# BolinLai/CSTS

Measured on AMD Instinct MI355X. Metric: clips/sec training (fwd+bwd) CSTS-Ego4D 16x256^2 bf16, higher is better.
Workload: dtype bf16; 1 GPU; CSTS_Ego4D_Gaze_Forecast.yaml train step (fwd + KLDiv + 0.05*EgoNCE + bwd + clip + AdamW), 16x256^2 video + 24 kHz STFT audio, b=4/GPU; mode=train, global_batch=4, frames=16, crop=256, parallelism=dp1, step=hip_graph, hip_graph=True, rccl_ranks=1

## Files before the change

### csts_amd/csrc/common.h

```cpp
#pragma once
#include <hip/hip_runtime.h>
#include <stdint.h>
#include <stddef.h>
#include <string>

#include "../../include/csts_hip.h"

#ifdef CSTS_HALF_F16
typedef _Float16 bf16;
typedef _Float16 bf16x8 __attribute__((ext_vector_type(8)));
typedef _Float16 bf16x4 __attribute__((ext_vector_type(4)));
typedef _Float16 bf16x2 __attribute__((ext_vector_type(2)));
#define CSTS_MFMA16 __builtin_amdgcn_mfma_f32_32x32x16_f16
#else
typedef __bf16 bf16;
typedef __bf16 bf16x8 __attribute__((ext_vector_type(8)));
typedef __bf16 bf16x4 __attribute__((ext_vector_type(4)));
typedef __bf16 bf16x2 __attribute__((ext_vector_type(2)));
#define CSTS_MFMA16 __builtin_amdgcn_mfma_f32_32x32x16_bf16
#endif
typedef short s16x4 __attribute__((ext_vector_type(4)));
typedef float f32x16 __attribute__((ext_vector_type(16)));
typedef float f32x4 __attribute__((ext_vector_type(4)));
typedef float f32x2 __attribute__((ext_vector_type(2)));

#define WAVE 64

__device__ __forceinline__ f32x4 ld_stream(const f32x4* p) {
#ifdef CSTS_NO_STREAM_POLICY
  return *p;
#else
  return __builtin_nontemporal_load(p);
#endif
}
__device__ __forceinline__ bf16x4 ld_stream(const bf16x4* p) {
#ifdef CSTS_NO_STREAM_POLICY
  return *p;
#else
  return __builtin_nontemporal_load(p);
#endif
}
__device__ __forceinline__ bf16x8 ld_stream(const bf16x8* p) {
#ifdef CSTS_NO_STREAM_POLICY
  return *p;
#else
  return __builtin_nontemporal_load(p);
#endif
}
typedef unsigned u32x4_t __attribute__((ext_vector_type(4)));
typedef unsigned u32x2_t __attribute__((ext_vector_type(2)));
struct StreamOut {
  __amdgpu_buffer_rsrc_t rsrc;
  __device__ __forceinline__ StreamOut(void* base, int64_t bytes) : rsrc(__builtin_amdgcn_make_buffer_rsrc(base, 0, (int)bytes, 0x00020000)) {}
  __device__ __forceinline__ void st16(int off, f32x4 v) const {
#ifdef CSTS_NO_STREAM_POLICY
    __builtin_amdgcn_raw_buffer_store_b128(__builtin_bit_cast(u32x4_t, v), rsrc, off, 0, 0);
#else
    __builtin_amdgcn_raw_buffer_store_b128(__builtin_bit_cast(u32x4_t, v), rsrc, off, 0, 17);
#endif
  }
  __device__ __forceinline__ void st8(int off, bf16x4 v) const {
#ifdef CSTS_NO_STREAM_POLICY
    __builtin_amdgcn_raw_buffer_store_b64(__builtin_bit_cast(u32x2_t, v), rsrc, off, 0, 0);
#else
    __builtin_amdgcn_raw_buffer_store_b64(__builtin_bit_cast(u32x2_t, v), rsrc, off, 0, 17);
#endif
  }
};

__device__ __forceinline__ float h16_lo(unsigned v) {
#ifdef CSTS_HALF_F16
  return (float)__builtin_bit_cast(_Float16, (unsigned short)(v & 0xffffu));
#else
  return __uint_as_float(v << 16);
#endif
}
__device__ __forceinline__ float h16_hi(unsigned v) {
#ifdef CSTS_HALF_F16
  return (float)__builtin_bit_cast(_Float16, (unsigned short)(v >> 16));
#else
  return __uint_as_float(v & 0xffff0000u);
#endif
}

void csts_set_error(const std::string& s);
#define CSTS_FAIL(msg)                                                         \
  do {                                                                         \
    csts_set_error(std::string(__func__) + ": " + (msg));                      \
    return -1;                                                                 \
  } while (0)
#define CSTS_REQUIRE(cond, msg)                                                \
  do {                                                                         \
    if (!(cond)) CSTS_FAIL(std::string(msg) + " [" #cond "]");                 \
  } while (0)
#define CSTS_LAUNCH_CHECK()                                                    \
  do {                                                                         \
    hipError_t e__ = hipGetLastError();                                        \
    if (e__ != hipSuccess) CSTS_FAIL(std::string("launch: ") + hipGetErrorString(e__)); \
  } while (0)

#include <map>
#include <mutex>
#include <utility>
static inline bool csts_dyn_lds_optin(const void* fn, int bytes) {
  static std::mutex mu;
  static std::map<std::pair<const void*, int>, int> done;
  int dev = 0;
  if (hipGetDevice(&dev) != hipSuccess) return false;
  std::lock_guard<std::mutex> lock(mu);
  auto it = done.find({fn, dev});
  if (it != done.end() && it->second >= bytes) return true;
  if (hipFuncSetAttribute(fn, hipFuncAttributeMaxDynamicSharedMemorySize, bytes) != hipSuccess) return false;
  done[{fn, dev}] = bytes;
  return true;
}

static inline bool aligned16(const void* p) { return (reinterpret_cast<uintptr_t>(p) & 15) == 0; }
static inline int64_t cdiv(int64_t a, int64_t b) { return (a + b - 1) / b; }

__device__ __forceinline__ float ld_as_f32(const void* p, int dt, int64_t i) {
  return dt == CSTS_F32 ? reinterpret_cast<const float*>(p)[i] : (float)reinterpret_cast<const bf16*>(p)[i];
}
__device__ __forceinline__ void st_from_f32(void* p, int dt, int64_t i, float v) {
  if (dt == CSTS_F32) reinterpret_cast<float*>(p)[i] = v;
  else reinterpret_cast<bf16*>(p)[i] = (bf16)v;
}

__device__ __forceinline__ void ld8_as_f32(const void* p, int dt, int64_t i, float (&o)[8]) {
  if (dt == CSTS_F32) {
    const float4* q = reinterpret_cast<const float4*>(reinterpret_cast<const float*>(p) + i);
    float4 a = q[0], b = q[1];
    o[0] = a.x; o[1] = a.y; o[2] = a.z; o[3] = a.w; o[4] = b.x; o[5] = b.y; o[6] = b.z; o[7] = b.w;
  } else {
    bf16x8 v = *reinterpret_cast<const bf16x8*>(reinterpret_cast<const bf16*>(p) + i);
#pragma unroll
    for (int j = 0; j < 8; ++j) o[j] = (float)v[j];
  }
}
__device__ __forceinline__ void st8_from_f32(void* p, int dt, int64_t i, const float (&o)[8]) {
  if (dt == CSTS_F32) {
    float4* q = reinterpret_cast<float4*>(reinterpret_cast<float*>(p) + i);
    q[0] = make_float4(o[0], o[1], o[2], o[3]);
    q[1] = make_float4(o[4], o[5], o[6], o[7]);
  } else {
    bf16x8 v;
#pragma unroll
    for (int j = 0; j < 8; ++j) v[j] = (bf16)o[j];
    *reinterpret_cast<bf16x8*>(reinterpret_cast<bf16*>(p) + i) = v;
  }
}

__device__ __forceinline__ float wave_sum(float v) {
#pragma unroll
  for (int o = 32; o > 0; o >>= 1) v += __shfl_xor(v, o, 64);
  return v;
}
__device__ __forceinline__ float wave_max(float v) {
#pragma unroll
  for (int o = 32; o > 0; o >>= 1) v = fmaxf(v, __shfl_xor(v, o, 64));
  return v;
}

__device__ __forceinline__ float gelu_f(float x) { return 0.5f * x * (1.0f + erff(x * 0.70710678118654752f)); }
__device__ __forceinline__ float dgelu_f(float x) {
  const float cdf = 0.5f * (1.0f + erff(x * 0.70710678118654752f));
  const float pdf = 0.39894228040143268f * __expf(-0.5f * x * x);
  return cdf + x * pdf;
}

__device__ __forceinline__ float erf_poly_times_exp(float ax, float e) {
  const float t = __builtin_amdgcn_rcpf(1.f + 0.3275911f * ax);
  const float poly = t * (0.254829592f + t * (-0.284496736f + t * (1.421413741f + t * (-1.453152027f + t * 1.061405429f))));
  return 1.f - poly * e;
}
__device__ __forceinline__ float gelu_fast(float x) {
  const float t = x * 0.70710678118654752f, ax = fabsf(t);
  const float e = __expf(-ax * ax);
  const float er = copysignf(erf_poly_times_exp(ax, e), x);
  return 0.5f * x * (1.0f + er);
}
__device__ __forceinline__ float dgelu_fast(float x) {
  const float t = x * 0.70710678118654752f, ax = fabsf(t);
  const float e = __expf(-ax * ax);
  const float er = copysignf(erf_poly_times_exp(ax, e), x);
  return 0.5f * (1.0f + er) + x * 0.39894228040143268f * e;
}

int csts_reduce_rows_launch(const float* ws, float* out, int64_t nrows, int64_t ncols, float scale, hipStream_t s);
```

### csts_amd/csrc/optim.hip

```cpp
#include "common.h"
#include <algorithm>
#include <type_traits>

namespace {

constexpr int OPT_THREADS = 256;
constexpr int OPT_VEC = 4;

struct OptTables {
  const int32_t* chunk_tensor;
  const int64_t* chunk_off;
  const csts_opt_tensor* tensors;
  const void* const* grads;
};

template <bool G16> __device__ __forceinline__ float ldg(const void* g, int64_t i) {
  if constexpr (G16) return (float)reinterpret_cast<const bf16*>(g)[i];
  else return reinterpret_cast<const float*>(g)[i];
}
template <bool G16> __device__ __forceinline__ float4 ldg4(const void* g, int64_t i4) {
  if constexpr (G16) {
    const bf16x4 v = ld_stream(reinterpret_cast<const bf16x4*>(g) + i4);
    return make_float4((float)v[0], (float)v[1], (float)v[2], (float)v[3]);
  } else {
    const f32x4 v = ld_stream(reinterpret_cast<const f32x4*>(g) + i4);
    return make_float4(v[0], v[1], v[2], v[3]);
  }
}
__device__ __forceinline__ float4 ld4s(const float* p, int64_t i4) {
  const f32x4 v = ld_stream(reinterpret_cast<const f32x4*>(p) + i4);
  return make_float4(v[0], v[1], v[2], v[3]);
}

template <bool G16>
__global__ __launch_bounds__(OPT_THREADS) void opt_sqnorm_kernel(OptTables t, int chunk_elems, float* __restrict__ partial,
                                                                 const float* __restrict__ scaler) {
  __shared__ float red[OPT_THREADS / WAVE];
  const int c = blockIdx.x;
  const int ti = t.chunk_tensor[c];
  const int64_t off = t.chunk_off[c];
  const char* g = reinterpret_cast<const char*>(t.grads[ti]);
  const float inv = scaler != nullptr ? 1.f / scaler[0] : 1.f;
  float s = 0.f;
  if (g != nullptr) {
    const int64_t n = min((int64_t)chunk_elems, t.tensors[ti].n - off);
    g += off * (G16 ? 2 : 4);
    const bool vec = (reinterpret_cast<uintptr_t>(g) & (G16 ? 7 : 15)) == 0;
    if (vec) {
      const int64_t n4 = n / OPT_VEC;
      for (int64_t i = threadIdx.x; i < n4; i += OPT_THREADS) {
        float4 v = ldg4<G16>(g, i);
        v.x *= inv; v.y *= inv; v.z *= inv; v.w *= inv;
        s += v.x * v.x + v.y * v.y + v.z * v.z + v.w * v.w;
      }
      for (int64_t i = n4 * OPT_VEC + threadIdx.x; i < n; i += OPT_THREADS) { const float x = ldg<G16>(g, i) * inv; s += x * x; }
    } else {
      for (int64_t i = threadIdx.x; i < n; i += OPT_THREADS) { const float x = ldg<G16>(g, i) * inv; s += x * x; }
    }
  }
  s = wave_sum(s);
  if ((threadIdx.x & 63) == 0) red[threadIdx.x >> 6] = s;
  __syncthreads();
  if (threadIdx.x == 0) {
    float tot = 0.f;
#pragma unroll
    for (int w = 0; w < OPT_THREADS / WAVE; ++w) tot += red[w];
    partial[c] = tot;
  }
}

__global__ __launch_bounds__(1024) void opt_norm_finish_kernel(const float* __restrict__ partial, int nchunks, float max_norm,
                                                               float* __restrict__ state, float* __restrict__ scaler, float growth,
                                                               float backoff, int growth_interval, const float* __restrict__ extra_sq,
                                                               int n_extra) {
  __shared__ float red[1024 / WAVE];
  float s = 0.f;
  for (int i = threadIdx.x; i < nchunks; i += 1024) s += partial[i];
  if (extra_sq != nullptr && (int)threadIdx.x < n_extra) {
    const float inv = scaler != nullptr ? 1.f / scaler[0] : 1.f;
    s += extra_sq[threadIdx.x] * inv * inv;
  }
  s = wave_sum(s);
  if ((threadIdx.x & 63) == 0) red[threadIdx.x >> 6] = s;
  __syncthreads();
  if (threadIdx.x == 0) {
    float tot = 0.f;
#pragma unroll
    for (int w = 0; w < 1024 / WAVE; ++w) tot += red[w];
    const float norm = sqrtf(tot);
    state[1] = norm;
    if (scaler != nullptr) {
      const float scale = scaler[0];
      const bool bad = !(norm == norm) || norm > 3.0e38f;
      if (bad) {
        state[2] = 0.f;
        state[3] = 1.f;
        scaler[0] = scale * backoff;
        scaler[1] = 0.f;
        return;
      }
      float tracker = scaler[1] + 1.f;
      if (tracker >= (float)growth_interval) { scaler[0] = scale * growth; tracker = 0.f; }
      scaler[1] = tracker;
      state[0] += 1.f;
      state[3] = 0.f;
      state[2] = (max_norm > 0.f ? fminf(1.f, max_norm / (norm + 1e-6f)) : 1.f) / scale;
      return;
    }
    state[0] += 1.f;
    state[3] = 0.f;
    state[2] = max_norm > 0.f ? fminf(1.f, max_norm / (norm + 1e-6f)) : 1.f;
  }
}

__device__ __forceinline__ void adamw_one(float& p, float g, float& m, float& v, float clip, float lr, float wd, float b1,
                                          float b2, float eps, float step_size, float rsqrt_bc2) {
  g *= clip;
  p -= lr * wd * p;
  m += (1.f - b1) * (g - m);
  v = b2 * v + (1.f - b2) * g * g;
  const float denom = sqrtf(v) * rsqrt_bc2 + eps;
  p -= step_size * (m / denom);
}

struct RuleK {
  float momentum, dampening;
  float clip_value;
  int nesterov;
  float* buf_step;
};

template <int R, bool VC>
__device__ __forceinline__ void rule_one(float& p, float g, float& m, float& v, float clip, float lr, float wd, float b1, float b2, float eps,
                                         float step_size, float rsqrt_bc2, const RuleK& r, bool first) {
  g *= clip;
  if constexpr (VC) g = g < -r.clip_value ? -r.clip_value : (g > r.clip_value ? r.clip_value : g);
  if constexpr (R == CSTS_OPT_ADAMW) {
    adamw_one(p, g, m, v, 1.f, lr, wd, b1, b2, eps, step_size, rsqrt_bc2);
  } else if constexpr (R == CSTS_OPT_ADAM) {
    g += wd * p;
    m += (1.f - b1) * (g - m);
    v = b2 * v + (1.f - b2) * g * g;
    const float denom = sqrtf(v) * rsqrt_bc2 + eps;
    p -= step_size * (m / denom);
  } else {
    float d = g + wd * p;
    if (r.momentum != 0.f) {
      m = first ? d : r.momentum * m + (1.f - r.dampening) * d;
      d = r.nesterov ? d + r.momentum * m : m;
    }
    p -= lr * d;
  }
}

template <int R> __device__ __forceinline__ bool rule_first(const RuleK& r, int ti, float step) {
  if constexpr (R != CSTS_OPT_SGD) return false;
  if (r.momentum == 0.f) return false;
  const float f = r.buf_step[ti];
  return f == 0.f || f == step;
}
template <int R> __device__ __forceinline__ void rule_mark(const RuleK& r, int ti, float step, bool first, bool leader) {
  if constexpr (R == CSTS_OPT_SGD) {
    if (first && leader) r.buf_step[ti] = step;
  }
}

template <bool G16, int R, bool VC>
__global__ __launch_bounds__(OPT_THREADS) void opt_adamw_kernel(OptTables t, int chunk_elems, const float* __restrict__ lr_ptr,
                                                                const float* __restrict__ state, float b1, float b2, float eps, RuleK rk) {
  const int c = blockIdx.x;
  const int ti = t.chunk_tensor[c];
  const char* g = reinterpret_cast<const char*>(t.grads[ti]);
  if (g == nullptr || state[3] != 0.f) return;
  const csts_opt_tensor tt = t.tensors[ti];
  const int64_t off = t.chunk_off[c];
  const int64_t n = min((int64_t)chunk_elems, tt.n - off);
  const float lr = *lr_ptr, step = state[0], clip = state[2];
  const float bc1 = 1.f - powf(b1, step), bc2 = 1.f - powf(b2, step);
  const float step_size = lr / bc1, rsqrt_bc2 = 1.f / sqrtf(bc2);
  constexpr bool USE_V = R != CSTS_OPT_SGD;
  const bool use_m = R != CSTS_OPT_SGD || rk.momentum != 0.f;
  if ((use_m && tt.m == nullptr) || (USE_V && tt.v == nullptr)) return;
  const bool first = rule_first<R>(rk, ti, step);
  float* p = reinterpret_cast<float*>(tt.p) + off;
  float* m = use_m ? reinterpret_cast<float*>(tt.m) + off : nullptr;
  float* v = USE_V ? reinterpret_cast<float*>(tt.v) + off : nullptr;
  bf16* w16 = tt.w16 ? reinterpret_cast<bf16*>(tt.w16) + off : nullptr;
  g += off * (G16 ? 2 : 4);
  const bool vec = ((reinterpret_cast<uintptr_t>(p) | reinterpret_cast<uintptr_t>(m) | reinterpret_cast<uintptr_t>(v)) & 15) == 0 &&
                   (reinterpret_cast<uintptr_t>(g) & (G16 ? 7 : 15)) == 0 && (w16 == nullptr || (reinterpret_cast<uintptr_t>(w16) & 7) == 0);
  int64_t done = 0;
  if (vec) {
    const int64_t n4 = n / OPT_VEC;
    const StreamOut sp(p, n * 4), sm(m ? (void*)m : (void*)p, n * 4), sv(v ? (void*)v : (void*)p, n * 4),
        sw(w16 ? (void*)w16 : (void*)p, n * 2);
    auto f4 = [](const float4& x) { f32x4 o; o[0] = x.x; o[1] = x.y; o[2] = x.z; o[3] = x.w; return o; };
    for (int64_t i = threadIdx.x; i < n4; i += OPT_THREADS) {
      float4 pp = ld4s(p, i);
      const float4 gg = ldg4<G16>(g, i);
      float4 mm = make_float4(0.f, 0.f, 0.f, 0.f), vv = mm;
      if (use_m && !first) mm = ld4s(m, i);
      if (USE_V) vv = ld4s(v, i);
      rule_one<R, VC>(pp.x, gg.x, mm.x, vv.x, clip, lr, tt.weight_decay, b1, b2, eps, step_size, rsqrt_bc2, rk, first);
      rule_one<R, VC>(pp.y, gg.y, mm.y, vv.y, clip, lr, tt.weight_decay, b1, b2, eps, step_size, rsqrt_bc2, rk, first);
      rule_one<R, VC>(pp.z, gg.z, mm.z, vv.z, clip, lr, tt.weight_decay, b1, b2, eps, step_size, rsqrt_bc2, rk, first);
      rule_one<R, VC>(pp.w, gg.w, mm.w, vv.w, clip, lr, tt.weight_decay, b1, b2, eps, step_size, rsqrt_bc2, rk, first);
      sp.st16((int)i * 16, f4(pp));
      if (use_m) sm.st16((int)i * 16, f4(mm));
      if (USE_V) sv.st16((int)i * 16, f4(vv));
      if (w16) {
        bf16x4 w;
        w[0] = (bf16)pp.x; w[1] = (bf16)pp.y; w[2] = (bf16)pp.z; w[3] = (bf16)pp.w;
        sw.st8((int)i * 8, w);
      }
    }
    done = n4 * OPT_VEC;
  }
  for (int64_t i = done + threadIdx.x; i < n; i += OPT_THREADS) {
    float pp = p[i], mm = use_m && !first ? m[i] : 0.f, vv = USE_V ? v[i] : 0.f;
    rule_one<R, VC>(pp, ldg<G16>(g, i), mm, vv, clip, lr, tt.weight_decay, b1, b2, eps, step_size, rsqrt_bc2, rk, first);
    p[i] = pp;
    if (use_m) m[i] = mm;
    if (USE_V) v[i] = vv;
    if (w16) w16[i] = (bf16)pp;
  }
  rule_mark<R>(rk, ti, step, first, off == 0 && threadIdx.x == 0);
}


constexpr int FK = 256;
constexpr int FT = 64;
constexpr int FMAX = 8;

struct FactoredList { csts_opt_factored it[FMAX]; int64_t ws_off[FMAX]; };

__device__ __forceinline__ float ld_a(const void* a, int a_dt, int64_t i) {
  return a_dt == CSTS_F32 ? reinterpret_cast<const float*>(a)[i] : (float)reinterpret_cast<const bf16*>(a)[i];
}

__global__ __launch_bounds__(256) void factored_gram_kernel(FactoredList l, float* __restrict__ ws) {
  extern __shared__ __attribute__((aligned(16))) float fsm[];
  float (*As)[FK + 1] = reinterpret_cast<float (*)[FK + 1]>(fsm);
  const csts_opt_factored& it = l.it[blockIdx.z];
  const int nslab = it.K / FK;
  if ((int)blockIdx.x >= nslab) return;
  const int k0 = blockIdx.x * FK, T = it.T;
  for (int i = threadIdx.x; i < T * (FK / 8); i += 256) {
    const int t = i / (FK / 8), k = (i - t * (FK / 8)) * 8;
    float v[8];
    ld8_as_f32(it.a, it.a_dt, (int64_t)t * it.K + k0 + k, v);
#pragma unroll
    for (int j = 0; j < 8; ++j) As[t][k + j] = v[j];
  }
  __syncthreads();
  float* out = ws + l.ws_off[blockIdx.z] + (int64_t)blockIdx.x * T * T;
  for (int pr = threadIdx.x; pr < T * T; pr += 256) {
    const int t = pr / T, u = pr - t * T;
    float s = 0.f;
#pragma unroll 8
    for (int k = 0; k < FK; ++k) s += As[t][k] * As[u][k];
    out[pr] = s;
  }
}
constexpr int FPARTS = 32;
__global__ __launch_bounds__(1024) void factored_sq_part_kernel(FactoredList l, const float* __restrict__ ws, float* __restrict__ parts) {
  const csts_opt_factored& it = l.it[blockIdx.y];
  const int T = it.T, nslab = it.K / FK, b = blockIdx.x;
  const float* w = ws + l.ws_off[blockIdx.y];
  float* out = parts + ((int64_t)blockIdx.y * FPARTS + b) * 2 * FT * FT;
  const int nb = (it.N + FPARTS - 1) / FPARTS, n_beg = b * nb, n_end = min(it.N, n_beg + nb);
  for (int pr = threadIdx.x; pr < T * T; pr += 1024) {
    const int t = pr / T, u = pr - t * T;
    float g2 = 0.f;
    for (int s = b; s < nslab; s += FPARTS) g2 += w[(int64_t)s * T * T + pr];
    float g1 = 0.f;
    if (it.a_dt == CSTS_F32) {
      for (int n = n_beg; n < n_end; ++n) g1 += it.dy[(int64_t)t * it.N + n] * it.dy[(int64_t)u * it.N + n];
    } else {
      for (int n = n_beg; n < n_end; ++n) g1 += (float)(bf16)it.dy[(int64_t)t * it.N + n] * (float)(bf16)it.dy[(int64_t)u * it.N + n];
    }
    out[pr] = g2;
    out[FT * FT + pr] = g1;
  }
}
__global__ __launch_bounds__(1024) void factored_sq_finish_kernel(FactoredList l, const float* __restrict__ parts, float* __restrict__ out_sq) {
  __shared__ float red[1024 / WAVE];
  const csts_opt_factored& it = l.it[blockIdx.x];
  const int T = it.T;
  const float* w = parts + (int64_t)blockIdx.x * FPARTS * 2 * FT * FT;
  float acc = 0.f;
  for (int pr = threadIdx.x; pr < T * T; pr += 1024) {
    float g2 = 0.f, g1 = 0.f;
    for (int b = 0; b < FPARTS; ++b) { g2 += w[(int64_t)b * 2 * FT * FT + pr]; g1 += w[(int64_t)b * 2 * FT * FT + FT * FT + pr]; }
    acc += g1 * g2;
  }
  acc = wave_sum(acc);
  if ((threadIdx.x & 63) == 0) red[threadIdx.x >> 6] = acc;
  __syncthreads();
  if (threadIdx.x == 0) {
    float tot = 0.f;
#pragma unroll
    for (int i = 0; i < 1024 / WAVE; ++i) tot += red[i];
    out_sq[blockIdx.x] = (tot == tot) ? fmaxf(tot, 0.f) : __builtin_inff();
  }
}
constexpr int FR = 32;
template <int R, bool VC>
__global__ __launch_bounds__(256) void opt_adamw_factored_kernel(FactoredList l, const float* __restrict__ lr_ptr,
                                                                 const float* __restrict__ state, float b1, float b2, float eps, RuleK rk) {
  extern __shared__ __attribute__((aligned(16))) float fsm[];
  if (state[3] != 0.f) return;
  const csts_opt_factored& it = l.it[blockIdx.z];
  float (*As)[FK] = reinterpret_cast<float (*)[FK]>(fsm);
  float (*Ds)[FR] = reinterpret_cast<float (*)[FR]>(fsm + it.T * FK);
  const int k0 = blockIdx.x * FK, n0 = blockIdx.y * FR, T = it.T;
  if (k0 >= it.K || n0 >= it.N) return;
  for (int i = threadIdx.x; i < T * (FK / 8); i += 256) {
    const int t = i / (FK / 8), k = (i - t * (FK / 8)) * 8;
    float v[8];
    ld8_as_f32(it.a, it.a_dt, (int64_t)t * it.K + k0 + k, v);
    *reinterpret_cast<float4*>(&As[t][k]) = make_float4(v[0], v[1], v[2], v[3]);
    *reinterpret_cast<float4*>(&As[t][k + 4]) = make_float4(v[4], v[5], v[6], v[7]);
  }
  for (int i = threadIdx.x; i < T * FR; i += 256) {
    const int t = i / FR, n = i - t * FR;
    Ds[t][n] = (n0 + n < it.N) ? it.dy[(int64_t)t * it.N + n0 + n] : 0.f;
  }
  __syncthreads();
  const float lr = *lr_ptr, step = state[0], clip = state[2];
  const float bc1 = 1.f - powf(b1, step), bc2 = 1.f - powf(b2, step);
  const float step_size = lr / bc1, rsqrt_bc2 = 1.f / sqrtf(bc2);
  const bool use_m = R != CSTS_OPT_SGD || rk.momentum != 0.f;
  constexpr bool USE_V = R != CSTS_OPT_SGD;
  const bool first = rule_first<R>(rk, it.tensor, step);
  const int kq = (threadIdx.x & 63) * 4;
  const int nr = threadIdx.x >> 6;
  constexpr int RPT = FR / 4;
  float g[RPT][4];
#pragma unroll
  for (int rr = 0; rr < RPT; ++rr) { g[rr][0] = 0.f; g[rr][1] = 0.f; g[rr][2] = 0.f; g[rr][3] = 0.f; }
  for (int t = 0; t < T; ++t) {
    const float4 av = *reinterpret_cast<const float4*>(&As[t][kq]);
#pragma unroll
    for (int rr = 0; rr < RPT; ++rr) {
      const float d = Ds[t][nr + 4 * rr];
      g[rr][0] += d * av.x; g[rr][1] += d * av.y; g[rr][2] += d * av.z; g[rr][3] += d * av.w;
    }
  }
#pragma unroll
  for (int rr = 0; rr < RPT; ++rr) {
    const int n = n0 + nr + 4 * rr;
    if (n >= it.N) continue;
    const int64_t at = (int64_t)n * it.K + k0 + kq;
    float4 pp = *reinterpret_cast<float4*>(it.p + at), mm = make_float4(0.f, 0.f, 0.f, 0.f), vv = mm;
    if (use_m && !first) mm = *reinterpret_cast<float4*>(it.m + at);
    if (USE_V) vv = *reinterpret_cast<float4*>(it.v + at);
    rule_one<R, VC>(pp.x, g[rr][0], mm.x, vv.x, clip, lr, it.weight_decay, b1, b2, eps, step_size, rsqrt_bc2, rk, first);
    rule_one<R, VC>(pp.y, g[rr][1], mm.y, vv.y, clip, lr, it.weight_decay, b1, b2, eps, step_size, rsqrt_bc2, rk, first);
    rule_one<R, VC>(pp.z, g[rr][2], mm.z, vv.z, clip, lr, it.weight_decay, b1, b2, eps, step_size, rsqrt_bc2, rk, first);
    rule_one<R, VC>(pp.w, g[rr][3], mm.w, vv.w, clip, lr, it.weight_decay, b1, b2, eps, step_size, rsqrt_bc2, rk, first);
    *reinterpret_cast<float4*>(it.p + at) = pp;
    if (use_m) *reinterpret_cast<float4*>(it.m + at) = mm;
    if (USE_V) *reinterpret_cast<float4*>(it.v + at) = vv;
    if (it.w16 != nullptr) {
      bf16x4 w;
      w[0] = (bf16)pp.x; w[1] = (bf16)pp.y; w[2] = (bf16)pp.z; w[3] = (bf16)pp.w;
      *reinterpret_cast<bf16x4*>(reinterpret_cast<bf16*>(it.w16) + at) = w;
    }
  }
  rule_mark<R>(rk, it.tensor, step, first, blockIdx.x == 0 && blockIdx.y == 0 && threadIdx.x == 0);
}

template <int R, bool VC>
__global__ __launch_bounds__(256) void opt_adamw_factored_mfma_kernel(FactoredList l, const float* __restrict__ lr_ptr,
                                                                      const float* __restrict__ state, float b1, float b2, float eps, RuleK rk) {
  if (state[3] != 0.f) return;
  const csts_opt_factored& it = l.it[blockIdx.z];
  const int lane = threadIdx.x & 63, wave = threadIdx.x >> 6;
  const int n0 = blockIdx.y * 32, k0 = blockIdx.x * FK + wave * 64;
  if (k0 >= it.K || n0 >= it.N) return;
  const int T = it.T, N = it.N, K = it.K;
  const bf16* __restrict__ a16 = reinterpret_cast<const bf16*>(it.a);
  f32x16 acc[2];
#pragma unroll
  for (int j = 0; j < 2; ++j)
#pragma unroll
    for (int r = 0; r < 16; ++r) acc[j][r] = 0.f;
  const int nl = n0 + (lane & 31), kl = k0 + (lane & 31);
  for (int t0 = 0; t0 < T; t0 += 16) {
    bf16x8 dv, a0, a1;
#pragma unroll
    for (int e = 0; e < 8; ++e) {
      const int t = t0 + 8 * (lane >> 5) + e;
      const bool ok = t < T;
      dv[e] = (bf16)((ok && nl < N) ? it.dy[(int64_t)t * N + nl] : 0.f);
      a0[e] = ok ? a16[(int64_t)t * K + kl] : (bf16)0.f;
      a1[e] = ok ? a16[(int64_t)t * K + kl + 32] : (bf16)0.f;
    }
    acc[0] = CSTS_MFMA16(dv, a0, acc[0], 0, 0, 0);
    acc[1] = CSTS_MFMA16(dv, a1, acc[1], 0, 0, 0);
  }
  const float lr = *lr_ptr, step = state[0], clip = state[2];
  const float bc1 = 1.f - powf(b1, step), bc2 = 1.f - powf(b2, step);
  const float step_size = lr / bc1, rsqrt_bc2 = 1.f / sqrtf(bc2);
#ifdef CSTS_NO_STREAM_POLICY
  constexpr int LD_AUX = 0, ST_AUX = 0;
#else
  constexpr int LD_AUX = 2, ST_AUX = 17;
#endif
  const bool use_m = R != CSTS_OPT_SGD || rk.momentum != 0.f;
  constexpr bool USE_V = R != CSTS_OPT_SGD;
  const bool first = rule_first<R>(rk, it.tensor, step);
  const int bytes = (int)((int64_t)N * K * 4);
  const auto rp = __builtin_amdgcn_make_buffer_rsrc(it.p, 0, bytes, 0x00020000),
             rm = __builtin_amdgcn_make_buffer_rsrc(use_m ? (void*)it.m : (void*)it.p, 0, bytes, 0x00020000),
             rv = __builtin_amdgcn_make_buffer_rsrc(USE_V ? (void*)it.v : (void*)it.p, 0, bytes, 0x00020000),
             rw = __builtin_amdgcn_make_buffer_rsrc(it.w16 != nullptr ? it.w16 : (void*)it.p, 0, bytes / 2, 0x00020000);
#pragma unroll
  for (int j = 0; j < 2; ++j) {
    float pp[16], mm[16], vv[16];
#pragma unroll
    for (int r = 0; r < 16; ++r) {
      const int n = n0 + (r & 3) + 8 * (r >> 2) + 4 * (lane >> 5);
      const int off = (n < N) ? (n * K + kl + 32 * j) * 4 : 0;
      pp[r] = __builtin_bit_cast(float, __builtin_amdgcn_raw_buffer_load_b32(rp, off, 0, LD_AUX));
      mm[r] = use_m && !first ? __builtin_bit_cast(float, __builtin_amdgcn_raw_buffer_load_b32(rm, off, 0, LD_AUX)) : 0.f;
      vv[r] = USE_V ? __builtin_bit_cast(float, __builtin_amdgcn_raw_buffer_load_b32(rv, off, 0, LD_AUX)) : 0.f;
    }
#pragma unroll
    for (int r = 0; r < 16; ++r) {
      const int n = n0 + (r & 3) + 8 * (r >> 2) + 4 * (lane >> 5);
      if (n >= N) continue;
      const int off = (n * K + kl + 32 * j) * 4;
      rule_one<R, VC>(pp[r], acc[j][r], mm[r], vv[r], clip, lr, it.weight_decay, b1, b2, eps, step_size, rsqrt_bc2, rk, first);
      __builtin_amdgcn_raw_buffer_store_b32(__builtin_bit_cast(unsigned, pp[r]), rp, off, 0, ST_AUX);
      if (use_m) __builtin_amdgcn_raw_buffer_store_b32(__builtin_bit_cast(unsigned, mm[r]), rm, off, 0, ST_AUX);
      if (USE_V) __builtin_amdgcn_raw_buffer_store_b32(__builtin_bit_cast(unsigned, vv[r]), rv, off, 0, ST_AUX);
      if (it.w16 != nullptr) __builtin_amdgcn_raw_buffer_store_b16(__builtin_bit_cast(unsigned short, (bf16)pp[r]), rw, off / 2, 0, ST_AUX);
    }
  }
  rule_mark<R>(rk, it.tensor, step, first, blockIdx.x == 0 && blockIdx.y == 0 && threadIdx.x == 0);
}

}

constexpr int FT_MFMA = 256;
static int factored_fill(const csts_opt_factored* items, int nitems, FactoredList& l, int* max_k, int* max_n, int max_t = FT,
                         bool need_m = true, bool need_v = true) {
  CSTS_REQUIRE(items != nullptr && nitems > 0 && nitems <= FMAX, "1 .. 8 items per call");
  *max_k = 0; *max_n = 0;
  int64_t off = 0;
  for (int i = 0; i < nitems; ++i) {
    const csts_opt_factored& it = items[i];
    CSTS_REQUIRE(it.p && (it.m || !need_m) && (it.v || !need_v) && it.dy && it.a, "null pointer");
    CSTS_REQUIRE(it.T > 0 && it.T <= max_t && it.K > 0 && it.K % FK == 0 && it.N > 0 && it.N % 16 == 0,
                 "T <= 64 (256 for the update with 16-bit operands), K % 256 == 0, N % 16 == 0");
    CSTS_REQUIRE(it.a_dt == CSTS_F32 || it.a_dt == CSTS_HALF, "bad a dtype");
    CSTS_REQUIRE(aligned16(it.p) && (!need_m || aligned16(it.m)) && (!need_v || aligned16(it.v)) && (it.w16 == nullptr || ((uintptr_t)it.w16 & 7) == 0), "alignment");
    l.it[i] = it;
    l.ws_off[i] = off;
    off += (int64_t)(it.K / FK) * it.T * it.T;
    *max_k = std::max(*max_k, it.K); *max_n = std::max(*max_n, it.N);
  }
  return 0;
}

extern "C" size_t csts_factored_sqnorm_workspace(const csts_opt_factored* items, int nitems) {
  if (items == nullptr || nitems <= 0 || nitems > FMAX) return 0;
  size_t b = 0;
  for (int i = 0; i < nitems; ++i) b += (size_t)(items[i].K / FK) * items[i].T * items[i].T * sizeof(float);
  return b + (size_t)nitems * FPARTS * 2 * FT * FT * sizeof(float);
}
extern "C" int csts_factored_sqnorm(const csts_opt_factored* items, int nitems, float* out_sq, void* workspace, size_t ws_bytes,
                                    hipStream_t stream) {
  FactoredList l;
  int mk, mn;
  if (int rc = factored_fill(items, nitems, l, &mk, &mn, FT, false, false)) return rc;
  CSTS_REQUIRE(out_sq != nullptr && workspace != nullptr && aligned16(workspace) && ws_bytes >= csts_factored_sqnorm_workspace(items, nitems), "workspace too small");
  float* slabs = reinterpret_cast<float*>(workspace);
  int mt = 0;
  for (int i = 0; i < nitems; ++i) mt = std::max(mt, items[i].T);
  const size_t sm = (size_t)mt * (FK + 1) * sizeof(float);
  CSTS_REQUIRE(sm <= 64 * 1024 || csts_dyn_lds_optin(reinterpret_cast<const void*>(&factored_gram_kernel), (int)sm), "LDS opt-in failed");
  hipLaunchKernelGGL(factored_gram_kernel, dim3((unsigned)(mk / FK), 1, (unsigned)nitems), dim3(256), sm, stream, l, slabs);
  CSTS_LAUNCH_CHECK();
  size_t slab_floats = 0;
  for (int i = 0; i < nitems; ++i) slab_floats += (size_t)(items[i].K / FK) * items[i].T * items[i].T;
  float* parts = slabs + slab_floats;
  hipLaunchKernelGGL(factored_sq_part_kernel, dim3(FPARTS, (unsigned)nitems), dim3(1024), 0, stream, l, (const float*)slabs, parts);
  CSTS_LAUNCH_CHECK();
  hipLaunchKernelGGL(factored_sq_finish_kernel, dim3((unsigned)nitems), dim3(1024), 0, stream, l, (const float*)parts, out_sq);
  CSTS_LAUNCH_CHECK();
  return 0;
}
static int rule_check(const csts_opt_rule* rule, RuleK* rk) {
  CSTS_REQUIRE(rule != nullptr, "null rule");
  CSTS_REQUIRE(rule->kind == CSTS_OPT_ADAMW || rule->kind == CSTS_OPT_ADAM || rule->kind == CSTS_OPT_SGD, "bad rule kind");
  CSTS_REQUIRE(rule->kind == CSTS_OPT_SGD || (rule->momentum == 0.f && rule->dampening == 0.f && rule->nesterov == 0),
               "momentum / dampening / nesterov belong to the SGD rule");
  CSTS_REQUIRE(rule->momentum >= 0.f && rule->dampening >= 0.f && rule->dampening <= 1.f, "bad momentum / dampening");
  CSTS_REQUIRE(!rule->nesterov || (rule->momentum > 0.f && rule->dampening == 0.f), "nesterov needs momentum and zero dampening");
  CSTS_REQUIRE(rule->clip_value == rule->clip_value, "bad clip_value");
  const bool sgd_m = rule->kind == CSTS_OPT_SGD && rule->momentum != 0.f;
  CSTS_REQUIRE(!sgd_m || rule->buf_step != nullptr, "SGD with momentum needs buf_step");
  *rk = RuleK{rule->momentum, rule->dampening, rule->clip_value > 0.f ? rule->clip_value : 0.f, rule->nesterov ? 1 : 0,
              sgd_m ? rule->buf_step : nullptr};
  return 0;
}
static bool rule_uses_m(const csts_opt_rule* rule) { return rule->kind != CSTS_OPT_SGD || rule->momentum != 0.f; }
static bool rule_uses_v(const csts_opt_rule* rule) { return rule->kind != CSTS_OPT_SGD; }

template <typename K3> static void launch_rule(int kind, bool vc, K3 k) {
  using VT = std::true_type;
  using VF = std::false_type;
  if (kind == CSTS_OPT_ADAMW) vc ? k(std::integral_constant<int, CSTS_OPT_ADAMW>{}, VT{}) : k(std::integral_constant<int, CSTS_OPT_ADAMW>{}, VF{});
  else if (kind == CSTS_OPT_ADAM) vc ? k(std::integral_constant<int, CSTS_OPT_ADAM>{}, VT{}) : k(std::integral_constant<int, CSTS_OPT_ADAM>{}, VF{});
  else vc ? k(std::integral_constant<int, CSTS_OPT_SGD>{}, VT{}) : k(std::integral_constant<int, CSTS_OPT_SGD>{}, VF{});
}

extern "C" int csts_opt_factored_step(const csts_opt_factored* items, int nitems, const csts_opt_rule* rule, const float* state,
                                      const float* lr, float beta1, float beta2, float eps, hipStream_t stream) {
  RuleK rk;
  if (int rc = rule_check(rule, &rk)) return rc;
  FactoredList l;
  int mk, mn;
  bool half_ops = items != nullptr && nitems > 0 && nitems <= FMAX;
  for (int i = 0; half_ops && i < nitems; ++i) half_ops = items[i].a_dt == CSTS_HALF && (int64_t)items[i].N * items[i].K * 4 < ((int64_t)1 << 31) && items[i].K % 64 == 0;
  if (int rc = factored_fill(items, nitems, l, &mk, &mn, half_ops ? FT_MFMA : FT, rule_uses_m(rule), rule_uses_v(rule))) return rc;
  CSTS_REQUIRE(state != nullptr && lr != nullptr, "null state");
  for (int i = 0; i < nitems; ++i) CSTS_REQUIRE(items[i].tensor >= 0, "bad item tensor index");
  int mt = 0;
  for (int i = 0; i < nitems; ++i) mt = std::max(mt, items[i].T);
  bool all16 = true;
  for (int i = 0; i < nitems; ++i) all16 = all16 && items[i].a_dt == CSTS_HALF && (int64_t)items[i].N * items[i].K * 4 < ((int64_t)1 << 31) && items[i].K % 64 == 0;
  if (all16) {
    launch_rule(rule->kind, rk.clip_value > 0.f, [&](auto R, auto V) {
      hipLaunchKernelGGL((opt_adamw_factored_mfma_kernel<decltype(R)::value, decltype(V)::value>), dim3((unsigned)(mk / FK), (unsigned)cdiv(mn, 32), (unsigned)nitems),
                         dim3(256), 0, stream, l, lr, state, beta1, beta2, eps, rk);
    });
    CSTS_LAUNCH_CHECK();
    return 0;
  }
  const size_t sm = (size_t)mt * (FK + FR) * sizeof(float);
  int rc = 0;
  launch_rule(rule->kind, rk.clip_value > 0.f, [&](auto R, auto V) {
    const void* fn = reinterpret_cast<const void*>(&opt_adamw_factored_kernel<decltype(R)::value, decltype(V)::value>);
    if (sm > 64 * 1024 && !csts_dyn_lds_optin(fn, (int)sm)) { rc = -1; return; }
    hipLaunchKernelGGL((opt_adamw_factored_kernel<decltype(R)::value, decltype(V)::value>), dim3((unsigned)(mk / FK), (unsigned)cdiv(mn, FR), (unsigned)nitems), dim3(256), sm,
                       stream, l, lr, state, beta1, beta2, eps, rk);
  });
  CSTS_REQUIRE(rc == 0, "LDS opt-in failed");
  CSTS_LAUNCH_CHECK();
  return 0;
}
extern "C" int csts_adamw_factored(const csts_opt_factored* items, int nitems, const float* state, const float* lr, float beta1,
                                   float beta2, float eps, hipStream_t stream) {
  const csts_opt_rule rule{CSTS_OPT_ADAMW, 0.f, 0.f, 0, 0.f, 0, nullptr};
  return csts_opt_factored_step(items, nitems, &rule, state, lr, beta1, beta2, eps, stream);
}

extern "C" int csts_opt_step(const csts_opt_args* a, const csts_opt_rule* rule, hipStream_t stream) {
  RuleK rk;
  if (int rc = rule_check(rule, &rk)) return rc;
  CSTS_REQUIRE(a != nullptr, "null args");
  CSTS_REQUIRE(a->nchunks > 0 && a->ntensors > 0 && a->chunk_elems > 0 && a->chunk_elems % 4 == 0 && a->chunk_elems <= (1 << 28), "bad chunking");
  CSTS_REQUIRE(a->chunk_tensor && a->chunk_off && a->tensors && a->grads, "null table");
  CSTS_REQUIRE(a->partial && a->state && a->lr, "null state");
  CSTS_REQUIRE(a->beta1 >= 0.f && a->beta1 < 1.f && a->beta2 >= 0.f && a->beta2 < 1.f && a->eps > 0.f, "bad hyper-parameters");
  CSTS_REQUIRE(a->grad_dt == CSTS_F32 || a->grad_dt == CSTS_HALF, "bad gradient dtype");
  CSTS_REQUIRE(a->n_extra_sq >= 0 && a->n_extra_sq <= 1024 && (a->n_extra_sq == 0 || a->extra_sq != nullptr), "bad extra_sq");
  CSTS_REQUIRE(a->scaler == nullptr || (a->growth > 1.f && a->backoff > 0.f && a->backoff < 1.f && a->growth_interval > 0), "bad loss-scaler parameters");
  CSTS_REQUIRE(!(rule->clip_value > 0.f && a->max_grad_norm > 0.f), "clip_value and max_grad_norm are exclusive (the reference's if / elif)");
  OptTables t{a->chunk_tensor, a->chunk_off, a->tensors, a->grads};
  const bool g16 = a->grad_dt != CSTS_F32;
  const dim3 grid((unsigned)a->nchunks), block(OPT_THREADS);
  if (g16) hipLaunchKernelGGL(opt_sqnorm_kernel<true>, grid, block, 0, stream, t, a->chunk_elems, a->partial, (const float*)a->scaler);
  else hipLaunchKernelGGL(opt_sqnorm_kernel<false>, grid, block, 0, stream, t, a->chunk_elems, a->partial, (const float*)a->scaler);
  CSTS_LAUNCH_CHECK();
  hipLaunchKernelGGL(opt_norm_finish_kernel, dim3(1), dim3(1024), 0, stream, a->partial, a->nchunks, a->max_grad_norm, a->state,
                     a->scaler, a->growth, a->backoff, a->growth_interval, a->extra_sq, a->n_extra_sq);
  CSTS_LAUNCH_CHECK();
  launch_rule(rule->kind, rk.clip_value > 0.f, [&](auto R, auto V) {
    constexpr int RR = decltype(R)::value;
    constexpr bool VV = decltype(V)::value;
    if (g16) hipLaunchKernelGGL((opt_adamw_kernel<true, RR, VV>), grid, block, 0, stream, t, a->chunk_elems, a->lr, a->state, a->beta1, a->beta2, a->eps, rk);
    else hipLaunchKernelGGL((opt_adamw_kernel<false, RR, VV>), grid, block, 0, stream, t, a->chunk_elems, a->lr, a->state, a->beta1, a->beta2, a->eps, rk);
  });
  CSTS_LAUNCH_CHECK();
  return 0;
}
extern "C" int csts_adamw_step(const csts_opt_args* a, hipStream_t stream) {
  const csts_opt_rule rule{CSTS_OPT_ADAMW, 0.f, 0.f, 0, 0.f, 0, nullptr};
  return csts_opt_step(a, &rule, stream);
}
```

Baseline: 206.7 clips/s.

## Add streaming factored AdamW kernel with LDS transpose and vectorized state I/O

Adds a new fused factored-gradient AdamW kernel, enabled by default, that transposes the MFMA accumulator through LDS. This lets each lane load and store param, m, v in 16-byte vector rows instead of scalar 4-byte accesses. It issues half the state loads before the MFMA loop, software-pipelines the operand loads across iterations, and pins occupancy at three waves per EU. It also relaxes the N alignment requirement to 8 and adds compile-time diagnostic switches to the old kernel. The cost is 32KB of LDS per block and higher register pressure. The optimizer is a small share of the whole training step.

After: 208.2 clips/s, median of 6. Within noise of the previous version (+0.7%).

```diff
diff --git a/csts_amd/csrc/common.h b/csts_amd/csrc/common.h
--- a/csts_amd/csrc/common.h
+++ b/csts_amd/csrc/common.h
@@ -57,6 +57,13 @@
     __builtin_amdgcn_raw_buffer_store_b128(__builtin_bit_cast(u32x4_t, v), rsrc, off, 0, 0);
 #else
     __builtin_amdgcn_raw_buffer_store_b128(__builtin_bit_cast(u32x4_t, v), rsrc, off, 0, 17);
+#endif
+  }
+  __device__ __forceinline__ f32x4 ld16(int off) const {
+#ifdef CSTS_NO_STREAM_POLICY
+    return __builtin_bit_cast(f32x4, __builtin_amdgcn_raw_buffer_load_b128(rsrc, off, 0, 0));
+#else
+    return __builtin_bit_cast(f32x4, __builtin_amdgcn_raw_buffer_load_b128(rsrc, off, 0, 2));
 #endif
   }
   __device__ __forceinline__ void st8(int off, bf16x4 v) const {
diff --git a/csts_amd/csrc/optim.hip b/csts_amd/csrc/optim.hip
--- a/csts_amd/csrc/optim.hip
+++ b/csts_amd/csrc/optim.hip
@@ -371,6 +371,9 @@
   rule_mark<R>(rk, it.tensor, step, first, blockIdx.x == 0 && blockIdx.y == 0 && threadIdx.x == 0);
 }
 
+#ifndef CSTS_FACT_DIAG
+#define CSTS_FACT_DIAG 0
+#endif
 template <int R, bool VC>
 __global__ __launch_bounds__(256) void opt_adamw_factored_mfma_kernel(FactoredList l, const float* __restrict__ lr_ptr,
                                                                       const float* __restrict__ state, float b1, float b2, float eps, RuleK rk) {
@@ -387,19 +390,6 @@
 #pragma unroll
     for (int r = 0; r < 16; ++r) acc[j][r] = 0.f;
   const int nl = n0 + (lane & 31), kl = k0 + (lane & 31);
-  for (int t0 = 0; t0 < T; t0 += 16) {
-    bf16x8 dv, a0, a1;
-#pragma unroll
-    for (int e = 0; e < 8; ++e) {
-      const int t = t0 + 8 * (lane >> 5) + e;
-      const bool ok = t < T;
-      dv[e] = (bf16)((ok && nl < N) ? it.dy[(int64_t)t * N + nl] : 0.f);
-      a0[e] = ok ? a16[(int64_t)t * K + kl] : (bf16)0.f;
-      a1[e] = ok ? a16[(int64_t)t * K + kl + 32] : (bf16)0.f;
-    }
-    acc[0] = CSTS_MFMA16(dv, a0, acc[0], 0, 0, 0);
-    acc[1] = CSTS_MFMA16(dv, a1, acc[1], 0, 0, 0);
-  }
   const float lr = *lr_ptr, step = state[0], clip = state[2];
   const float bc1 = 1.f - powf(b1, step), bc2 = 1.f - powf(b2, step);
   const float step_size = lr / bc1, rsqrt_bc2 = 1.f / sqrtf(bc2);
@@ -416,16 +406,48 @@
              rm = __builtin_amdgcn_make_buffer_rsrc(use_m ? (void*)it.m : (void*)it.p, 0, bytes, 0x00020000),
              rv = __builtin_amdgcn_make_buffer_rsrc(USE_V ? (void*)it.v : (void*)it.p, 0, bytes, 0x00020000),
              rw = __builtin_amdgcn_make_buffer_rsrc(it.w16 != nullptr ? it.w16 : (void*)it.p, 0, bytes / 2, 0x00020000);
+#if CSTS_FACT_DIAG & 4
+  float hp[2][16], hm[2][16], hv[2][16];
+#pragma unroll
+  for (int j = 0; j < 2; ++j)
+#pragma unroll
+    for (int r = 0; r < 16; ++r) {
+      const int n = n0 + (r & 3) + 8 * (r >> 2) + 4 * (lane >> 5);
+      const int off = (n < N) ? (n * K + kl + 32 * j) * 4 : 0;
+      hp[j][r] = __builtin_bit_cast(float, __builtin_amdgcn_raw_buffer_load_b32(rp, off, 0, LD_AUX));
+      hm[j][r] = use_m && !first ? __builtin_bit_cast(float, __builtin_amdgcn_raw_buffer_load_b32(rm, off, 0, LD_AUX)) : 0.f;
+      hv[j][r] = USE_V ? __builtin_bit_cast(float, __builtin_amdgcn_raw_buffer_load_b32(rv, off, 0, LD_AUX)) : 0.f;
+    }
+#endif
+#if !(CSTS_FACT_DIAG & 1)
+  for (int t0 = 0; t0 < T; t0 += 16) {
+    bf16x8 dv, a0, a1;
+#pragma unroll
+    for (int e = 0; e < 8; ++e) {
+      const int t = t0 + 8 * (lane >> 5) + e;
+      const bool ok = t < T;
+      dv[e] = (bf16)((ok && nl < N) ? it.dy[(int64_t)t * N + nl] : 0.f);
+      a0[e] = ok ? a16[(int64_t)t * K + kl] : (bf16)0.f;
+      a1[e] = ok ? a16[(int64_t)t * K + kl + 32] : (bf16)0.f;
+    }
+    acc[0] = CSTS_MFMA16(dv, a0, acc[0], 0, 0, 0);
+    acc[1] = CSTS_MFMA16(dv, a1, acc[1], 0, 0, 0);
+  }
+#endif
 #pragma unroll
   for (int j = 0; j < 2; ++j) {
     float pp[16], mm[16], vv[16];
 #pragma unroll
     for (int r = 0; r < 16; ++r) {
+#if CSTS_FACT_DIAG & 4
+      pp[r] = hp[j][r]; mm[r] = hm[j][r]; vv[r] = hv[j][r];
+#else
       const int n = n0 + (r & 3) + 8 * (r >> 2) + 4 * (lane >> 5);
       const int off = (n < N) ? (n * K + kl + 32 * j) * 4 : 0;
       pp[r] = __builtin_bit_cast(float, __builtin_amdgcn_raw_buffer_load_b32(rp, off, 0, LD_AUX));
       mm[r] = use_m && !first ? __builtin_bit_cast(float, __builtin_amdgcn_raw_buffer_load_b32(rm, off, 0, LD_AUX)) : 0.f;
       vv[r] = USE_V ? __builtin_bit_cast(float, __builtin_amdgcn_raw_buffer_load_b32(rv, off, 0, LD_AUX)) : 0.f;
+#endif
     }
 #pragma unroll
     for (int r = 0; r < 16; ++r) {
@@ -436,7 +458,102 @@
       __builtin_amdgcn_raw_buffer_store_b32(__builtin_bit_cast(unsigned, pp[r]), rp, off, 0, ST_AUX);
       if (use_m) __builtin_amdgcn_raw_buffer_store_b32(__builtin_bit_cast(unsigned, mm[r]), rm, off, 0, ST_AUX);
       if (USE_V) __builtin_amdgcn_raw_buffer_store_b32(__builtin_bit_cast(unsigned, vv[r]), rv, off, 0, ST_AUX);
+#if !(CSTS_FACT_DIAG & 2)
       if (it.w16 != nullptr) __builtin_amdgcn_raw_buffer_store_b16(__builtin_bit_cast(unsigned short, (bf16)pp[r]), rw, off / 2, 0, ST_AUX);
+#endif
+    }
+  }
+  rule_mark<R>(rk, it.tensor, step, first, blockIdx.x == 0 && blockIdx.y == 0 && threadIdx.x == 0);
+}
+
+template <int R, bool VC>
+__global__ __launch_bounds__(256) __attribute__((amdgpu_waves_per_eu(3, 3))) void opt_adamw_factored_mfma_stream_kernel(FactoredList l, const float* __restrict__ lr_ptr,
+                                                                             const float* __restrict__ state, float b1, float b2, float eps, RuleK rk) {
+  __shared__ __attribute__((aligned(16))) float slab[4][32 * 64];
+  if (state[3] != 0.f) return;
+  const csts_opt_factored& it = l.it[blockIdx.z];
+  const int lane = threadIdx.x & 63, wave = threadIdx.x >> 6;
+  const int n0 = blockIdx.y * 32, k0 = blockIdx.x * FK + wave * 64;
+  if (k0 >= it.K || n0 >= it.N) return;
+  const int T = it.T, N = it.N, K = it.K;
+  const bf16* __restrict__ a16 = reinterpret_cast<const bf16*>(it.a);
+  const int nl = n0 + (lane & 31), kl = k0 + (lane & 31);
+  auto operands = [&](int t0, bf16x8& dv, bf16x8& a0, bf16x8& a1) {
+#pragma unroll
+    for (int e = 0; e < 8; ++e) {
+      const int t = t0 + 8 * (lane >> 5) + e;
+      const bool ok = t < T;
+      dv[e] = (bf16)((ok && nl < N) ? it.dy[(int64_t)t * N + nl] : 0.f);
+      a0[e] = ok ? a16[(int64_t)t * K + kl] : (bf16)0.f;
+      a1[e] = ok ? a16[(int64_t)t * K + kl + 32] : (bf16)0.f;
+    }
+  };
+  bf16x8 dv, a0, a1;
+  operands(0, dv, a0, a1);
+  const float lr = *lr_ptr, step = state[0], clip = state[2];
+  const bool use_m = R != CSTS_OPT_SGD || rk.momentum != 0.f;
+  constexpr bool USE_V = R != CSTS_OPT_SGD;
+  const bool first = rule_first<R>(rk, it.tensor, step);
+  const int bytes = (int)((int64_t)N * K * 4);
+  const StreamOut sp(it.p, bytes), sm(use_m ? (void*)it.m : (void*)it.p, bytes), sv(USE_V ? (void*)it.v : (void*)it.p, bytes),
+      sw(it.w16 != nullptr ? it.w16 : (void*)it.p, bytes / 2);
+  const int nr = n0 + (lane >> 4), kc = k0 + 4 * (lane & 15);
+  f32x4 pp[8], mm[8], vv[8];
+  constexpr int EARLY = 4;
+  auto load_rows = [&](auto I0, auto I1) {
+#pragma unroll
+    for (int i = decltype(I0)::value; i < decltype(I1)::value; ++i) {
+      const int off = (nr + 4 * i < N) ? ((nr + 4 * i) * K + kc) * 4 : 0;
+      pp[i] = sp.ld16(off);
+      if (use_m && !first) mm[i] = sm.ld16(off);
+      else mm[i] = f32x4{0.f, 0.f, 0.f, 0.f};
+      if (USE_V) vv[i] = sv.ld16(off);
+      else vv[i] = f32x4{0.f, 0.f, 0.f, 0.f};
+    }
+  };
+  load_rows(std::integral_constant<int, 0>{}, std::integral_constant<int, EARLY>{});
+  f32x16 acc[2];
+#pragma unroll
+  for (int j = 0; j < 2; ++j)
+#pragma unroll
+    for (int r = 0; r < 16; ++r) acc[j][r] = 0.f;
+  for (int t0 = 0; t0 < T; t0 += 16) {
+    bf16x8 dn = dv, an0 = a0, an1 = a1;
+    if (t0 + 16 < T) operands(t0 + 16, dn, an0, an1);
+    acc[0] = CSTS_MFMA16(dv, a0, acc[0], 0, 0, 0);
+    acc[1] = CSTS_MFMA16(dv, a1, acc[1], 0, 0, 0);
+    dv = dn; a0 = an0; a1 = an1;
+  }
+  load_rows(std::integral_constant<int, EARLY>{}, std::integral_constant<int, 8>{});
+  float* sl = slab[wave];
+#pragma unroll
+  for (int j = 0; j < 2; ++j)
+#pragma unroll
+    for (int r = 0; r < 16; ++r) sl[((r & 3) + 8 * (r >> 2) + 4 * (lane >> 5)) * 64 + (lane & 31) + 32 * j] = acc[j][r];
+  __builtin_amdgcn_fence(__ATOMIC_RELEASE, "wavefront");
+  __builtin_amdgcn_wave_barrier();
+  __builtin_amdgcn_fence(__ATOMIC_ACQUIRE, "wavefront");
+  const float bc1 = 1.f - powf(b1, step), bc2 = 1.f - powf(b2, step);
+  const float step_size = lr / bc1, rsqrt_bc2 = 1.f / sqrtf(bc2);
+#pragma unroll
+  for (int i = 0; i < 8; ++i) {
+    const int n = nr + 4 * i;
+    if (n >= N) continue;
+    const f32x4 g = *reinterpret_cast<const f32x4*>(sl + (4 * i + (lane >> 4)) * 64 + 4 * (lane & 15));
+    const int off = (n * K + kc) * 4;
+#pragma unroll
+    for (int c = 0; c < 4; ++c) {
+      float p1 = pp[i][c], m1 = mm[i][c], v1 = vv[i][c];
+      rule_one<R, VC>(p1, g[c], m1, v1, clip, lr, it.weight_decay, b1, b2, eps, step_size, rsqrt_bc2, rk, first);
+      pp[i][c] = p1; mm[i][c] = m1; vv[i][c] = v1;
+    }
+    sp.st16(off, pp[i]);
+    if (use_m) sm.st16(off, mm[i]);
+    if (USE_V) sv.st16(off, vv[i]);
+    if (it.w16 != nullptr) {
+      bf16x4 w;
+      w[0] = (bf16)pp[i][0]; w[1] = (bf16)pp[i][1]; w[2] = (bf16)pp[i][2]; w[3] = (bf16)pp[i][3];
+      sw.st8(off / 2, w);
     }
   }
   rule_mark<R>(rk, it.tensor, step, first, blockIdx.x == 0 && blockIdx.y == 0 && threadIdx.x == 0);
@@ -453,8 +570,8 @@
   for (int i = 0; i < nitems; ++i) {
     const csts_opt_factored& it = items[i];
     CSTS_REQUIRE(it.p && (it.m || !need_m) && (it.v || !need_v) && it.dy && it.a, "null pointer");
-    CSTS_REQUIRE(it.T > 0 && it.T <= max_t && it.K > 0 && it.K % FK == 0 && it.N > 0 && it.N % 16 == 0,
-                 "T <= 64 (256 for the update with 16-bit operands), K % 256 == 0, N % 16 == 0");
+    CSTS_REQUIRE(it.T > 0 && it.T <= max_t && it.K > 0 && it.K % FK == 0 && it.N > 0 && it.N % 8 == 0,
+                 "T <= 64 (256 for the update with 16-bit operands), K % 256 == 0, N % 8 == 0");
     CSTS_REQUIRE(it.a_dt == CSTS_F32 || it.a_dt == CSTS_HALF, "bad a dtype");
     CSTS_REQUIRE(aligned16(it.p) && (!need_m || aligned16(it.m)) && (!need_v || aligned16(it.v)) && (it.w16 == nullptr || ((uintptr_t)it.w16 & 7) == 0), "alignment");
     l.it[i] = it;
@@ -534,9 +651,11 @@
   bool all16 = true;
   for (int i = 0; i < nitems; ++i) all16 = all16 && items[i].a_dt == CSTS_HALF && (int64_t)items[i].N * items[i].K * 4 < ((int64_t)1 << 31) && items[i].K % 64 == 0;
   if (all16) {
+    static const bool stream_form = [] { const char* e = getenv("CSTS_FACTORED_STREAM"); return !(e && e[0] == '0') && CSTS_FACT_DIAG == 0; }();
+    const dim3 grid((unsigned)(mk / FK), (unsigned)cdiv(mn, 32), (unsigned)nitems);
     launch_rule(rule->kind, rk.clip_value > 0.f, [&](auto R, auto V) {
-      hipLaunchKernelGGL((opt_adamw_factored_mfma_kernel<decltype(R)::value, decltype(V)::value>), dim3((unsigned)(mk / FK), (unsigned)cdiv(mn, 32), (unsigned)nitems),
-                         dim3(256), 0, stream, l, lr, state, beta1, beta2, eps, rk);
+      if (stream_form) hipLaunchKernelGGL((opt_adamw_factored_mfma_stream_kernel<decltype(R)::value, decltype(V)::value>), grid, dim3(256), 0, stream, l, lr, state, beta1, beta2, eps, rk);
+      else hipLaunchKernelGGL((opt_adamw_factored_mfma_kernel<decltype(R)::value, decltype(V)::value>), grid, dim3(256), 0, stream, l, lr, state, beta1, beta2, eps, rk);
     });
     CSTS_LAUNCH_CHECK();
     return 0;
```
